# rodrigo-paganini/kalman-vae

Hardware: AMD Instinct MI355X
Metric: sequences/sec (ELBO training step, 32x32xT bouncing-ball) (higher is better)
Workload: dtype f32; 1 GPU; BASELINE configs[1] (configs[2] per-GPU shard): bouncing-ball 32x32, T=50, batch=256/GPU, dynamics=lstm K=3, z=4, u=4, a=2, full train step (fwd incl. sigmoid(x_logits) + loss incl. active-unit stats + bwd + clip + Adam); both the GPU leg and the cpu_baseline leg do this work; preset=c2, global_batch=256, seq_len=50, parallelism=dp1, capture=hipgraph, loss_finite=True, dist_backend=none

## Files before the change

kalman-vae_amd/csrc/kvae_vae.hip:

```cpp
#include <hip/hip_runtime.h>

#include <stdint.h>
#include <stdio.h>
#include <stdlib.h>
#include <string.h>

#include "../../include/kvae_lgssm.h"

namespace kvae {}
using namespace kvae;

extern "C" int kvae_launch_status(const char *what);
static int launch_status(const char *what) { return kvae_launch_status(what); }

#include "vae_epilogue.h"

__device__ __forceinline__ void colsum_v4_body(const float *__restrict__ partials, float *__restrict__ out, int64_t rows, int64_t cols,
                                               unsigned block) {
  __shared__ float4 red[8][64];
  const int lane = threadIdx.x & 63, wv = threadIdx.x >> 6;
  const int64_t c = ((int64_t)block * 64 + lane) * 4;
  float4 s0 = make_float4(0.f, 0.f, 0.f, 0.f), s1 = s0, s2 = s0, s3 = s0;
  if (c < cols) {
    const float *p = partials + c;
// ... 86 lines not shown
    epi_fwd_elem(s, in, bias, out, o, relu);
}

__global__ __launch_bounds__(256) void k_vae_epilogue_bwd_bias(const float *__restrict__ g_out, const float *__restrict__ out,
                                                               float *__restrict__ g_in, float *__restrict__ bias_partials,
                                                               EpiShape s, int n_per_chunk, int relu) {
  extern __shared__ float bins[];
  const int Cin = s.C * s.r * s.r;
  const int OW = s.W * s.r, OH = s.H * s.r;
  const int64_t vol = (int64_t)s.C * OH * OW;
  for (int i = threadIdx.x; i < Cin; i += 256) bins[i] = 0.f;
  __syncthreads();
  const int64_t pos = (int64_t)blockIdx.x * 256 + threadIdx.x;
  if (pos < vol) {
    const int ow = (int)(pos % OW);
    const int oh = (int)((pos / OW) % OH);
    const int c = (int)(pos / ((int64_t)OW * OH));
    const int ch = c * s.r * s.r + (oh % s.r) * s.r + (ow % s.r);
    const int64_t in_off = ((int64_t)ch * s.H + oh / s.r) * s.W + ow / s.r;
    const int64_t in_vol = (int64_t)Cin * s.H * s.W;
    const int64_t n0 = (int64_t)blockIdx.y * n_per_chunk;
    const int64_t n1 = n0 + n_per_chunk < s.N ? n0 + n_per_chunk : s.N;
    float acc = 0.f;
    for (int64_t n = n0; n < n1; ++n) {
      float g = g_out[n * vol + pos];
      if (relu && !(out[n * vol + pos] > 0.f)) g = 0.f;
      g_in[n * in_vol + in_off] = g;
      acc += g;
    }
    atomicAdd(&bins[ch], acc);
  }
  __syncthreads();
  for (int i = threadIdx.x; i < Cin; i += 256) {
    if (bins[i] != 0.f) atomicAdd(&bias_partials[(int64_t)blockIdx.y * Cin + i], bins[i]);
  }
}

__global__ __launch_bounds__(256) void k_vae_epilogue_bwd(const float *g_out, const float *out, float *g_in, EpiShape s,
                                                          int64_t total, int relu) {
  for (int64_t o = (int64_t)blockIdx.x * 256 + threadIdx.x; o < total; o += (int64_t)gridDim.x * 256)
    epi_bwd_elem(s, g_out, out, g_in, o, relu);
}

#define KVAE_EPI_SAMPLES_PER_CHUNK 32
extern "C" int64_t kvae_bias_partial_rows(int64_t N);
static unsigned epi_grid(int64_t total) {
  const int64_t blocks = (total + 255) / 256;
  return (unsigned)(blocks < 256 * 32 ? blocks : 256 * 32);
}

extern "C" {
int kvae_bias_shuffle_act_fwd(const float *in, const float *bias, float *out, int64_t N, int32_t C, int32_t H, int32_t W,
                              int32_t r, int32_t relu, void *stream) {
  if (!in || !bias || !out) return KVAE_ERR_NULL;
  if (N < 1 || C < 1 || H < 1 || W < 1 || r < 1) return KVAE_ERR_ARG;
  const EpiShape s{N, C, H, W, r};
  const int64_t total = N * C * H * W * r * r;
  const bool aligned = ((uintptr_t)in % 16 == 0) && ((uintptr_t)out % 16 == 0);
  if (aligned && r == 1 && W % 4 == 0)
    k_vae_epilogue_fwd_v4<1><<<dim3(epi_grid(total / 4)), dim3(256), 0, (hipStream_t)stream>>>(in, bias, out, C, H, W, total / 4, relu);
  else if (aligned && r == 2 && W % 2 == 0)
    k_vae_epilogue_fwd_v4<2><<<dim3(epi_grid(total / 4)), dim3(256), 0, (hipStream_t)stream>>>(in, bias, out, C, H, W, total / 4, relu);
  else
    k_vae_epilogue_fwd<<<dim3(epi_grid(total)), dim3(256), 0, (hipStream_t)stream>>>(in, bias, out, s, total, relu);
  return launch_status("k_vae_epilogue_fwd");
}
int kvae_bias_shuffle_act_bwd(const float *g_out, const float *out, float *g_in, float *bias_partials, int64_t N, int32_t C,
                              int32_t H, int32_t W, int32_t r, int32_t relu, void *stream) {
  if (!g_out || !g_in || (relu && !out)) return KVAE_ERR_NULL;
  if (N < 1 || C < 1 || H < 1 || W < 1 || r < 1) return KVAE_ERR_ARG;
  const EpiShape s{N, C, H, W, r};
  const int64_t total = N * C * H * W * r * r;
  hipStream_t st = (hipStream_t)stream;
  if (bias_partials) {
    const int Cin = C * r * r;
    const int64_t chunks = kvae_bias_partial_rows(N);
    if (hipMemsetAsync(bias_partials, 0, sizeof(float) * chunks * Cin, st) != hipSuccess) return launch_status("memset bias_partials");
    const int64_t vol = (int64_t)C * H * W * r * r;
    k_vae_epilogue_bwd_bias<<<dim3((unsigned)((vol + 255) / 256), (unsigned)chunks), dim3(256), sizeof(float) * Cin, st>>>(
        g_out, out, g_in, bias_partials, s, KVAE_EPI_SAMPLES_PER_CHUNK, relu);
    return launch_status("k_vae_epilogue_bwd_bias");
  }
  k_vae_epilogue_bwd<<<dim3(epi_grid(total)), dim3(256), 0, st>>>(g_out, out, g_in, s, total, relu);
  return launch_status("k_vae_epilogue_bwd");
}
int kvae_colsum(const float *partials, float *out, int64_t rows, int64_t cols, void *stream) {
  if (!partials || !out) return KVAE_ERR_NULL;
  if (rows < 1 || cols < 1) return KVAE_ERR_ARG;
  if ((cols & 3) == 0 && ((((uintptr_t)partials | (uintptr_t)out) & 15) == 0))
    k_colsum_v4<<<dim3((unsigned)((cols + 255) / 256)), dim3(512), 0, (hipStream_t)stream>>>(partials, out, rows, cols);
  else
    k_colsum<<<dim3((unsigned)((cols + 63) / 64)), dim3(256), 0, (hipStream_t)stream>>>(partials, out, rows, cols);
  return launch_status("k_colsum");
}
int kvae_colsum2(const float *pa, float *oa, int64_t rows_a, int64_t cols_a, const float *pb, float *ob, int64_t rows_b,
                 int64_t cols_b, void *stream) {
  if (!pa || !oa || !pb || !ob) return KVAE_ERR_NULL;
  if (rows_a < 1 || cols_a < 1 || rows_b < 1 || cols_b < 1) return KVAE_ERR_ARG;
  if (((cols_a | cols_b) & 3) == 0 && ((((uintptr_t)pa | (uintptr_t)oa | (uintptr_t)pb | (uintptr_t)ob) & 15) == 0)) {
    const unsigned nb_a = (unsigned)((cols_a + 255) / 256), nb_b = (unsigned)((cols_b + 255) / 256);
    k_colsum_v4_pair<<<dim3(nb_a + nb_b), dim3(512), 0, (hipStream_t)stream>>>(pa, oa, rows_a, cols_a, nb_a, pb, ob, rows_b, cols_b);
    return launch_status("k_colsum_v4_pair");
  }
  const int rc = kvae_colsum(pa, oa, rows_a, cols_a, stream);
  return rc ? rc : kvae_colsum(pb, ob, rows_b, cols_b, stream);
}
int64_t kvae_bias_partial_rows(int64_t N) { return (N + KVAE_EPI_SAMPLES_PER_CHUNK - 1) / KVAE_EPI_SAMPLES_PER_CHUNK; }
}

constexpr int CA_BLOCKS = 512;
constexpr int CA_MAX_SEG = 1024;
__global__ __launch_bounds__(256) void k_grad_sumsq(const float *__restrict__ g, int64_t n, const int32_t *__restrict__ seg_of,
                                                    int n_seg, const float *__restrict__ seg_active,
                                                    const float *__restrict__ div_dev, float *__restrict__ seg_steps,
                                                    float *__restrict__ ws) {
  __shared__ float red[256];
  const float inv = div_dev ? 1.0f / fmaxf(*div_dev, 1.0f) : 1.0f;
  const bool gated = seg_of && seg_active;
  float s = 0.f;
  for (int64_t i = (int64_t)blockIdx.x * 256 + threadIdx.x; i < n; i += (int64_t)gridDim.x * 256) {
    float v = g[i] * inv;
    if (gated && seg_active[seg_of[i]] == 0.f) v = 0.f;
    s = fmaf(v, v, s);
  }
  red[threadIdx.x] = s;
  __syncthreads();
  for (int o = 128; o > 0; o >>= 1) {
    if ((int)threadIdx.x < o) red[threadIdx.x] += red[threadIdx.x + o];
    __syncthreads();
  }
  if (threadIdx.x == 0) ws[blockIdx.x] = red[0];
  if (blockIdx.x == 0)
    for (int sg = threadIdx.x; sg < n_seg; sg += 256)
      if (!seg_active || seg_active[sg] != 0.f) seg_steps[sg] += 1.0f;
}
__global__ __launch_bounds__(256) void k_clip_adam(float *__restrict__ p, const float *__restrict__ g, float *__restrict__ m,
                                                   float *__restrict__ v, int64_t n, const int32_t *__restrict__ seg_of, int n_seg,
                                                   const float *__restrict__ seg_active, const float *__restrict__ seg_steps,
                                                   const float *__restrict__ lr_dev, float lr, float beta1, float beta2, float eps,
                                                   float wd, float clip, const float *__restrict__ div_dev,
                                                   float *__restrict__ norm_out, const float *__restrict__ ws, int nparts) {
  __shared__ float red[256];
  __shared__ float s_step_size[CA_MAX_SEG], s_bc2s[CA_MAX_SEG];
  float s = 0.f;
  for (int i = threadIdx.x; i < nparts; i += 256) s += ws[i];
  red[threadIdx.x] = s;
  const float lrv = lr_dev ? *lr_dev : lr;
  for (int sg = threadIdx.x; sg < n_seg; sg += 256) {
    const float step = seg_steps[sg];
    const bool on = !seg_active || seg_active[sg] != 0.f;
    s_step_size[sg] = on ? lrv / (1.0f - powf(beta1, step)) : -1.0f;
    s_bc2s[sg] = on ? sqrtf(1.0f - powf(beta2, step)) : 1.0f;
  }
  __syncthreads();
  for (int o = 128; o > 0; o >>= 1) {
    if ((int)threadIdx.x < o) red[threadIdx.x] += red[threadIdx.x + o];
    __syncthreads();
  }
  const float total = sqrtf(red[0]);
  if (norm_out && blockIdx.x == 0 && threadIdx.x == 0) *norm_out = total;
  const float inv = div_dev ? 1.0f / fmaxf(*div_dev, 1.0f) : 1.0f;
  const float scale = inv * (clip > 0.f ? fminf(clip / (total + 1e-6f), 1.0f) : 1.0f);
  for (int64_t i = (int64_t)blockIdx.x * 256 + threadIdx.x; i < n; i += (int64_t)gridDim.x * 256) {
    const int sg = seg_of ? seg_of[i] : 0;
    const float step_size = s_step_size[sg], bc2s = s_bc2s[sg];
    if (step_size < 0.f) continue;
    float gi = g[i] * scale;
    const float pi = p[i];
    if (wd != 0.f) gi = fmaf(wd, pi, gi);
    const float mi = m[i] + (gi - m[i]) * (1.0f - beta1);
    const float vi = beta2 * v[i] + (1.0f - beta2) * gi * gi;
    m[i] = mi, v[i] = vi;
    p[i] = pi - step_size * mi / (sqrtf(vi) / bc2s + eps);
  }
}
extern "C" int kvae_clip_adam(float *params, const float *grads, float *exp_avg, float *exp_avg_sq, int64_t n,
                              const int32_t *seg_of, int32_t n_seg, const float *seg_active, float *seg_steps, const float *lr_dev,
                              float lr, float beta1, float beta2, float eps, float weight_decay, float clip, const float *div_dev,
                              float *norm_out, float *ws, void *stream) {
  if (!params || !grads || !exp_avg || !exp_avg_sq || !seg_steps || !ws) return KVAE_ERR_NULL;
  if (n < 1 || n_seg < 1 || n_seg > CA_MAX_SEG || (!seg_of && n_seg != 1)) return KVAE_ERR_ARG;
  const int64_t want = (n + 1023) / 1024;
  const unsigned parts = (unsigned)(want < CA_BLOCKS ? want : CA_BLOCKS);
  k_grad_sumsq<<<dim3(parts), dim3(256), 0, (hipStream_t)stream>>>(grads, n, seg_of, n_seg, seg_active, div_dev, seg_steps, ws);
  int rc = launch_status("k_grad_sumsq");
  if (rc) return rc;
  const unsigned blocks = (unsigned)((n + 255) / 256 < 2048 ? (n + 255) / 256 : 2048);
  k_clip_adam<<<dim3(blocks), dim3(256), 0, (hipStream_t)stream>>>(params, grads, exp_avg, exp_avg_sq, n, seg_of, n_seg, seg_active,
                                                                   seg_steps, lr_dev, lr, beta1, beta2, eps, weight_decay, clip,
                                                                   div_dev, norm_out, ws, (int)parts);
  return launch_status("k_clip_adam");
}

#include "vae_loss.h"

__global__ __launch_bounds__(256) void k_vae_bce_fwd(const float *__restrict__ logits, const float *__restrict__ x,
                                                     float *__restrict__ frame_ll, int64_t frames, int pixels) {
  const int64_t f = (int64_t)blockIdx.x * 4 + (threadIdx.x >> 6);
  const int lane = threadIdx.x & 63;
  if (f >= frames) return;
  const float *l = logits + f * pixels, *t = x + f * pixels;
  float acc = 0.f;
  if ((pixels & 3) == 0 && (((uintptr_t)l | (uintptr_t)t) & 15) == 0) {
    for (int i = lane * 4; i < pixels; i += 256) {
      const float4 a = *reinterpret_cast<const float4 *>(l + i), b = *reinterpret_cast<const float4 *>(t + i);
      acc += bce_logit(a.x, b.x) + bce_logit(a.y, b.y) + bce_logit(a.z, b.z) + bce_logit(a.w, b.w);
    }
  } else {
    for (int i = lane; i < pixels; i += 64) acc += bce_logit(l[i], t[i]);
  }
  for (int off = 32; off > 0; off >>= 1) acc += __shfl_down(acc, off, 64);
  if (lane == 0) frame_ll[f] = -acc;
}

__global__ __launch_bounds__(256) void k_vae_bce_bwd(const float *__restrict__ logits, const float *__restrict__ x,
                                                     const float *__restrict__ g_frame, float *__restrict__ g_logits,
                                                     int64_t total, int pixels) {
  for (int64_t i = ((int64_t)blockIdx.x * 256 + threadIdx.x) * 4; i < total; i += (int64_t)gridDim.x * 1024) {
    const float g = -g_frame[i / pixels];
    const float4 a = *reinterpret_cast<const float4 *>(logits + i), b = *reinterpret_cast<const float4 *>(x + i);
    *reinterpret_cast<float4 *>(g_logits + i) = make_float4(g * (sigmoid_stable(a.x) - b.x), g * (sigmoid_stable(a.y) - b.y),
                                                            g * (sigmoid_stable(a.z) - b.z), g * (sigmoid_stable(a.w) - b.w));
  }
}
__global__ __launch_bounds__(256) void k_vae_bce_bwd_scalar(const float *logits, const float *x, const float *g_frame,
                                                            float *g_logits, int64_t total, int pixels) {
  for (int64_t i = (int64_t)blockIdx.x * 256 + threadIdx.x; i < total; i += (int64_t)gridDim.x * 256)
    g_logits[i] = -g_frame[i / pixels] * (sigmoid_stable(logits[i]) - x[i]);
}

extern "C" {
int kvae_bce_frames_fwd(const float *logits, const float *x, float *frame_ll, int64_t frames, int32_t pixels, void *stream) {
  if (!logits || !x || !frame_ll) return KVAE_ERR_NULL;
  if (frames < 1 || pixels < 1) return KVAE_ERR_ARG;
  k_vae_bce_fwd<<<dim3((unsigned)((frames + 3) / 4)), dim3(256), 0, (hipStream_t)stream>>>(logits, x, frame_ll, frames, pixels);
  return launch_status("k_vae_bce_fwd");
}
int kvae_bce_frames_bwd(const float *logits, const float *x, const float *g_frame, float *g_logits, int64_t frames,
                        int32_t pixels, void *stream) {
  if (!logits || !x || !g_frame || !g_logits) return KVAE_ERR_NULL;
  if (frames < 1 || pixels < 1) return KVAE_ERR_ARG;
  const int64_t total = frames * pixels;
  const bool v4 = (pixels & 3) == 0 && ((((uintptr_t)logits | (uintptr_t)x | (uintptr_t)g_logits) & 15) == 0);
  if (v4)
    k_vae_bce_bwd<<<dim3(epi_grid(total / 4)), dim3(256), 0, (hipStream_t)stream>>>(logits, x, g_frame, g_logits, total, pixels);
  else
    k_vae_bce_bwd_scalar<<<dim3(epi_grid(total)), dim3(256), 0, (hipStream_t)stream>>>(logits, x, g_frame, g_logits, total, pixels);
  return launch_status("k_vae_bce_bwd");
}
}

#include "vae_conv_edge.h"
extern "C" {
int64_t kvae_conv_edge_partial_rows(int64_t N) { return N < 1024 ? (N < 1 ? 1 : N) : 1024; }

int kvae_dec_head_fwd(const float *in, const float *W, const float *bias, float *logits, float *w_scratch, int64_t N,
                      int32_t Cin, int32_t side, void *stream) {
  if (!in || !W || !bias || !logits || !w_scratch) return KVAE_ERR_NULL;
  if (N < 1) return KVAE_ERR_ARG;
  if (Cin != DH_CI || side != DH_S) return KVAE_ERR_DIMS;
  k_dec_head_prep<<<dim3(1), dim3(256), 0, (hipStream_t)stream>>>(W, w_scratch);
  k_dec_head_fwd<<<dim3((unsigned)N), dim3(256), 0, (hipStream_t)stream>>>(in, w_scratch, bias, logits);
  return launch_status("k_dec_head_fwd");
}
int kvae_dec_head_bwd(const float *in, const float *W, const float *g_logits, float *g_in, float *w_partials,
                      float *b_partials, float *w_scratch, int64_t N, int32_t Cin, int32_t side, void *stream) {
  if (!in || !W || !g_logits || !w_partials || !b_partials || !w_scratch) return KVAE_ERR_NULL;
  if (N < 1) return KVAE_ERR_ARG;
  if (Cin != DH_CI || side != DH_S) return KVAE_ERR_DIMS;
  if (g_in) {
    k_dec_head_prep<<<dim3(1), dim3(256), 0, (hipStream_t)stream>>>(W, w_scratch);
    k_dec_head_bwd_data<<<dim3((unsigned)N), dim3(256), 0, (hipStream_t)stream>>>(g_logits, w_scratch, g_in);
    const int rc = launch_status("k_dec_head_bwd_data");
    if (rc) return rc;
  }
  k_dec_head_wrw<<<dim3((unsigned)kvae_conv_edge_partial_rows(N)), dim3(256), 0, (hipStream_t)stream>>>(in, g_logits, w_partials,
                                                                                                     b_partials, N);
  return launch_status("k_dec_head_wrw");
}
int kvae_enc_stem_fwd(const float *x, const float *W, const float *bias, float *out, uint32_t *relu_bits, int64_t N, int32_t Cout,
                      int32_t side, void *stream) {
  if (!x || !W || !bias || !out) return KVAE_ERR_NULL;
  if (N < 1) return KVAE_ERR_ARG;
  if (Cout != ES_CO || side != ES_IN) return KVAE_ERR_DIMS;
  k_enc_stem_fwd<<<dim3((unsigned)N), dim3(256), 0, (hipStream_t)stream>>>(x, W, bias, out, relu_bits);
  return launch_status("k_enc_stem_fwd");
}
int kvae_enc_stem_bwd(const float *x, const float *out, const uint32_t *relu_bits, const float *g_out, float *w_partials,
                      float *b_partials, int64_t N, int32_t Cout, int32_t side, void *stream) {
  if (!x || (!out && !relu_bits) || !g_out || !w_partials || !b_partials) return KVAE_ERR_NULL;
  if (N < 1) return KVAE_ERR_ARG;
  if (Cout != ES_CO || side != ES_IN) return KVAE_ERR_DIMS;
  static const int mfma = getenv("KVAE_STEM_MFMA") ? atoi(getenv("KVAE_STEM_MFMA")) : 1;
  const dim3 grid((unsigned)kvae_conv_edge_partial_rows(N));
  if (mfma == 1 && relu_bits) k_enc_stem_wrw_mfma<true><<<grid, dim3(256), 0, (hipStream_t)stream>>>(x, out, relu_bits, g_out, w_partials, b_partials, N);
  else if (!out) return KVAE_ERR_NULL;
  else if (mfma) k_enc_stem_wrw_mfma<false><<<grid, dim3(256), 0, (hipStream_t)stream>>>(x, out, relu_bits, g_out, w_partials, b_partials, N);
  else k_enc_stem_wrw<<<grid, dim3(256), 0, (hipStream_t)stream>>>(x, out, g_out, w_partials, b_partials, N);
  return launch_status("k_enc_stem_wrw");
}
}

#include "vae_conv_mid.h"
static inline int64_t enc_mid_grid(int64_t N, int32_t side) {
  const int64_t fpi = side == 16 ? 2 : 8, iters = (N + fpi - 1) / fpi;
  return iters < 256 ? (iters < 1 ? 1 : iters) : 256;
}
extern "C" {
int64_t kvae_enc_mid_partial_rows(int64_t N, int32_t side) { return enc_mid_grid(N, side); }

int kvae_enc_mid_fwd(const float *in, const float *W, const float *bias, float *out, int64_t N, int32_t C, int32_t side,
                     void *stream) {
  if (!in || !W || !bias || !out) return KVAE_ERR_NULL;
  if (N < 1 || (N + 256 * 8) * EM_C * side * side * 4 >= EM_MAX_BYTES) return KVAE_ERR_ARG;
  if (C != EM_C || (side != 16 && side != 8)) return KVAE_ERR_DIMS;
  const dim3 grid((unsigned)enc_mid_grid(N, side));
  if (side == 16) k_enc_mid_fwd<16><<<grid, dim3(256), 0, (hipStream_t)stream>>>(in, W, bias, out, N);
  else k_enc_mid_fwd<8><<<grid, dim3(256), 0, (hipStream_t)stream>>>(in, W, bias, out, N);
  return launch_status("k_enc_mid_fwd");
}
int kvae_enc_mid_bwd(const float *in, const float *W, const float *out, const float *g_out, float *g_in,
                     float *w_partials, float *b_partials, int64_t N, int32_t C, int32_t side, void *stream) {
  if (!in || !W || !out || !g_out || !w_partials || !b_partials) return KVAE_ERR_NULL;
  if (N < 1 || (N + 256 * 8) * EM_C * side * side * 4 >= EM_MAX_BYTES) return KVAE_ERR_ARG;
  if (C != EM_C || (side != 16 && side != 8)) return KVAE_ERR_DIMS;
  const dim3 grid((unsigned)enc_mid_grid(N, side));
  if (g_in) {
    if (side == 16) k_enc_mid_bwd_data<16><<<grid, dim3(256), 0, (hipStream_t)stream>>>(W, out, g_out, g_in, N);
    else k_enc_mid_bwd_data<8><<<grid, dim3(256), 0, (hipStream_t)stream>>>(W, out, g_out, g_in, N);
    const int rc = launch_status("k_enc_mid_bwd_data");
    if (rc) return rc;
  }
  if (side == 16) k_enc_mid_wrw<16><<<grid, dim3(256), 0, (hipStream_t)stream>>>(in, out, g_out, w_partials, b_partials, N);
  else k_enc_mid_wrw<8><<<grid, dim3(256), 0, (hipStream_t)stream>>>(in, out, g_out, w_partials, b_partials, N);
  return launch_status("k_enc_mid_wrw");
}
}

#include "vae_conv_up_wino.h"
static bool dec_up_wino() {
  static const int env = getenv("KVAE_WINO") ? atoi(getenv("KVAE_WINO")) : 1;
  return env != 0;
}
static int g_dec_up_wgs = 0;
static inline int64_t dec_up_cap() {
  static const int env = getenv("KVAE_UP_WGS") ? atoi(getenv("KVAE_UP_WGS")) : 0;
  const int v = env >= 1 && env <= 256 ? env : __atomic_load_n(&g_dec_up_wgs, __ATOMIC_RELAXED);
  return v >= 1 && v <= 256 ? v : 256;
}
static inline int64_t dec_up_grid(int64_t N, int32_t side) {
  const int64_t fpi = side == 8 ? 2 : 8, iters = (N + fpi - 1) / fpi, cap = dec_up_cap();
  return iters < cap ? (iters < 1 ? 1 : iters) : cap;
}
extern "C" {
int64_t kvae_dec_up_partial_rows(int64_t N, int32_t side) { return dec_up_grid(N, side); }
int32_t kvae_dec_up_set_workgroups(int32_t n) {
  const int32_t prev = (int32_t)dec_up_cap();
  __atomic_store_n(&g_dec_up_wgs, n >= 1 && n <= 256 ? n : 0, __ATOMIC_RELAXED);
  return prev;
}

int kvae_dec_up_fwd(const float *x, const float *W, const float *bias, float *out, int64_t N, int32_t Cin, int32_t side,
                    void *stream) {
  if (!x || !W || !bias || !out) return KVAE_ERR_NULL;
  if (N < 1 || (N + 256 * 8) * UP_CO * side * side * 4 >= EM_MAX_BYTES) return KVAE_ERR_ARG;
  if (Cin != UP_CI || (side != 8 && side != 4)) return KVAE_ERR_DIMS;
  const dim3 grid((unsigned)dec_up_grid(N, side));
  if (dec_up_wino()) {
    const int64_t sets = side == 8 ? N : (N + 3) / 4;
    const dim3 wgrid((unsigned)(sets < dec_up_cap() ? sets : dec_up_cap()));
    if (side == 8) k_dec_up_fwd_wino<8><<<wgrid, dim3(512), 0, (hipStream_t)stream>>>(x, W, bias, out, N);
    else k_dec_up_fwd_wino<4><<<wgrid, dim3(512), 0, (hipStream_t)stream>>>(x, W, bias, out, N);
    return launch_status("k_dec_up_fwd_wino");
  }
  if (side == 8) k_dec_up_fwd<8><<<grid, dim3(256), 0, (hipStream_t)stream>>>(x, W, bias, out, N);
  else k_dec_up_fwd<4><<<grid, dim3(256), 0, (hipStream_t)stream>>>(x, W, bias, out, N);
  return launch_status("k_dec_up_fwd");
}
int kvae_dec_up_bwd(const float *x, const float *W, const float *out, const float *g_out, float *g_x, float *w_partials,
                    float *b_partials, int64_t N, int32_t Cin, int32_t side, void *stream) {
  if (!x || !W || !out || !g_out || !w_partials || !b_partials) return KVAE_ERR_NULL;
  if (N < 1 || (N + 256 * 8) * UP_CO * side * side * 4 >= EM_MAX_BYTES) return KVAE_ERR_ARG;
  if (Cin != UP_CI || (side != 8 && side != 4)) return KVAE_ERR_DIMS;
  const dim3 grid((unsigned)dec_up_grid(N, side));
  if (g_x) {
    const int64_t sets = side == 8 ? N : (N + 3) / 4;
    const dim3 wgrid((unsigned)(sets < dec_up_cap() ? sets : dec_up_cap()));
    if (dec_up_wino() && side == 8) k_dec_up_bwd_data_wino<8><<<wgrid, dim3(512), 0, (hipStream_t)stream>>>(W, out, g_out, g_x, N);
    else if (dec_up_wino()) k_dec_up_bwd_data_wino<4><<<wgrid, dim3(512), 0, (hipStream_t)stream>>>(W, out, g_out, g_x, N);
    else if (side == 8) k_dec_up_bwd_data<8><<<grid, dim3(256), 0, (hipStream_t)stream>>>(W, out, g_out, g_x, N);
    else k_dec_up_bwd_data<4><<<grid, dim3(256), 0, (hipStream_t)stream>>>(W, out, g_out, g_x, N);
    const int rc = launch_status("k_dec_up_bwd_data");
    if (rc) return rc;
  }
  if (dec_up_wino()) {
    if (side == 8) k_dec_up_wrw_wino<8><<<grid, dim3(512), 0, (hipStream_t)stream>>>(x, out, g_out, w_partials, b_partials, N);
    else k_dec_up_wrw_wino<4><<<grid, dim3(512), 0, (hipStream_t)stream>>>(x, out, g_out, w_partials, b_partials, N);
    return launch_status("k_dec_up_wrw_wino");
  }
  if (side == 8) k_dec_up_wrw<8><<<grid, dim3(256), 0, (hipStream_t)stream>>>(x, out, g_out, w_partials, b_partials, N);
  else k_dec_up_wrw<4><<<grid, dim3(256), 0, (hipStream_t)stream>>>(x, out, g_out, w_partials, b_partials, N);
  return launch_status("k_dec_up_wrw");
}
}

#include "vae_heads.h"
extern "C" {
int64_t kvae_head_partial_rows(void) { return HD_WAVES; }

int kvae_enc_head_fwd(const float *feat, const float *Wmu, const float *bmu, const float *Wvar, const float *bvar,
                      const float *eps, float *mu, float *var, float *a, int64_t N, int32_t F, int32_t A,
                      float noise_emission, void *stream) {
  if (!feat || !Wmu || !bmu || !Wvar || !bvar || !mu || !var || !a) return KVAE_ERR_NULL;
  if (N < 1) return KVAE_ERR_ARG;
  if (F != HD_F || A != HD_A) return KVAE_ERR_DIMS;
  const unsigned grid = (unsigned)(N < 4 * 512 ? (N + 3) / 4 : 512);
  k_enc_head_fwd<<<dim3(grid), dim3(256), 0, (hipStream_t)stream>>>(feat, Wmu, bmu, Wvar, bvar, eps, noise_emission, mu, var, a, N);
  return launch_status("k_enc_head_fwd");
}
int kvae_enc_head_bwd(const float *feat, const float *Wmu, const float *Wvar, const float *var, const float *eps,
                      const float *g_a, const float *g_mu, const float *g_var, float *g_feat, float *w_partials,
                      float *b_partials, int64_t N, int32_t F, int32_t A, float noise_emission, void *stream) {
  if (!feat || !Wmu || !Wvar || !var || !g_feat || !w_partials || !b_partials) return KVAE_ERR_NULL;
  if (N < 1) return KVAE_ERR_ARG;
  if (F != HD_F || A != HD_A) return KVAE_ERR_DIMS;
  k_enc_head_bwd<<<dim3(HD_WAVES / 4), dim3(256), 0, (hipStream_t)stream>>>(feat, Wmu, Wvar, var, eps, g_a, g_mu, g_var,
                                                                             noise_emission, g_feat, w_partials, b_partials, N);
  return launch_status("k_enc_head_bwd");
}
int kvae_dec_fc_fwd(const float *a, const float *W, const float *b, float *h, int64_t N, int32_t F, int32_t A, void *stream) {
  if (!a || !W || !b || !h) return KVAE_ERR_NULL;
  if (N < 1) return KVAE_ERR_ARG;
  if (F != HD_F || A != HD_A) return KVAE_ERR_DIMS;
  k_dec_fc_fwd<<<dim3(epi_grid(N * (HD_F / 4))), dim3(256), 0, (hipStream_t)stream>>>(a, W, b, h, N * (HD_F / 4));
  return launch_status("k_dec_fc_fwd");
}
int kvae_dec_fc_bwd(const float *g_h, const float *a, const float *W, float *g_a, float *w_partials, float *b_partials,
                    int64_t N, int32_t F, int32_t A, void *stream) {
  if (!g_h || !a || !W || !g_a || !w_partials || !b_partials) return KVAE_ERR_NULL;
  if (N < 1) return KVAE_ERR_ARG;
  if (F != HD_F || A != HD_A) return KVAE_ERR_DIMS;
  k_dec_fc_bwd<<<dim3(HD_WAVES / 4), dim3(256), 0, (hipStream_t)stream>>>(g_h, a, W, g_a, w_partials, b_partials, N);
  return launch_status("k_dec_fc_bwd");
}
int kvae_latent_reg_fwd(const float *a, const float *mu, const float *var, float *reg, int64_t N, int32_t A, void *stream) {
  if (!a || !mu || !var || !reg) return KVAE_ERR_NULL;
  if (N < 1 || A < 1) return KVAE_ERR_ARG;
  k_latent_reg_fwd<<<dim3(epi_grid(N)), dim3(256), 0, (hipStream_t)stream>>>(a, mu, var, reg, N, A);
  return launch_status("k_latent_reg_fwd");
}
int kvae_latent_reg_bwd(const float *a, const float *mu, const float *var, const float *g, float *g_a, float *g_mu,
                        float *g_var, int64_t N, int32_t A, void *stream) {
  if (!a || !mu || !var || !g || !g_a || !g_mu || !g_var) return KVAE_ERR_NULL;
  if (N < 1 || A < 1) return KVAE_ERR_ARG;
  k_latent_reg_bwd<<<dim3(epi_grid(N * A)), dim3(256), 0, (hipStream_t)stream>>>(a, mu, var, g, g_a, g_mu, g_var, N, A);
  return launch_status("k_latent_reg_bwd");
}
int kvae_loss_head_fwd(const float *lpx, const float *regf, const float *mask, const float *elbo_kf, const float *beta,
                       float scale_reconstruction, float vae_weight, float kf_weight, const float *weights_dev, float *out6,
                       float *coef3, int64_t n, void *stream) {
  if (!lpx || !regf || !elbo_kf || !beta || !out6 || !coef3) return KVAE_ERR_NULL;
  if (n < 1) return KVAE_ERR_ARG;
  k_loss_head_fwd<<<dim3(1), dim3(1024), 0, (hipStream_t)stream>>>(lpx, regf, mask, elbo_kf, beta, scale_reconstruction, vae_weight,
                                                                  kf_weight, weights_dev, out6, coef3, n);
  return launch_status("k_loss_head_fwd");
}
int kvae_loss_head_bwd(const float *g_loss, const float *coef3, const float *mask, float *g_lpx, float *g_regf,
                       float *g_elbo_kf, int64_t n, void *stream) {
  if (!g_loss || !coef3 || !g_lpx || !g_regf || !g_elbo_kf) return KVAE_ERR_NULL;
  if (n < 1) return KVAE_ERR_ARG;
  k_loss_head_bwd<<<dim3(epi_grid(n)), dim3(256), 0, (hipStream_t)stream>>>(g_loss, coef3, mask, g_lpx, g_regf,
                                                                            g_elbo_kf, n);
  return launch_status("k_loss_head_bwd");
}
}
```

kalman-vae_amd/csrc/vae_conv_mid.h:

```cpp
#pragma once
#include <hip/hip_runtime.h>
#include <stdint.h>

namespace kvae {

typedef float em_f16 __attribute__((ext_vector_type(16)));
constexpr int EM_C = 32, EM_W = EM_C * EM_C * 9;

template <int S>
struct EmDims {
  static constexpr int OS = S / 2, PF = OS * OS;
  static constexpr int FPI = 128 / PF;
  static constexpr int PLANE = S * S, FRAME = EM_C * PLANE;
  static constexpr int IT_IN = FPI * FRAME;
  static constexpr int IT_OUT = FPI * EM_C * PF;
};

__device__ __forceinline__ void em_load_weights(float *Wl, const float *__restrict__ W, bool m_is_co) {
  for (int i = threadIdx.x; i < EM_W; i += 256) {
    const int tap = i >> 10, k = (i >> 5) & 31, m = i & 31;
    const int co = m_is_co ? m : k, ci = m_is_co ? k : m;
    Wl[i] = W[(co * EM_C + ci) * 9 + tap];
  }
}

constexpr int EM_OOB = 1 << 24;
constexpr int64_t EM_MAX_BYTES = (int64_t)1 << 31;

typedef unsigned int em_u4 __attribute__((ext_vector_type(4)));
__device__ __forceinline__ __amdgpu_buffer_rsrc_t em_rsrc(const void *p, int64_t bytes) {
  return __builtin_amdgcn_make_buffer_rsrc(const_cast<void *>(p), 0, (int)bytes, 0x00020000);
}
__device__ __forceinline__ float4 em_ld4(__amdgpu_buffer_rsrc_t r, uint32_t byte_off) {
  const em_u4 v = __builtin_amdgcn_raw_buffer_load_b128(r, byte_off, 0, 0);
  return make_float4(__uint_as_float(v.x), __uint_as_float(v.y), __uint_as_float(v.z), __uint_as_float(v.w));
}
__device__ __forceinline__ void em_st4(__amdgpu_buffer_rsrc_t r, uint32_t byte_off, const float4 v) {
  const em_u4 u = {__float_as_uint(v.x), __float_as_uint(v.y), __float_as_uint(v.z), __float_as_uint(v.w)};
  __builtin_amdgcn_raw_buffer_store_b128(u, r, byte_off, 0, 0);
}
__device__ __forceinline__ void em_st1(__amdgpu_buffer_rsrc_t r, uint32_t byte_off, float v) {
  __builtin_amdgcn_raw_buffer_store_b32(__float_as_uint(v), r, byte_off, 0, 0);
}
#ifdef KVAE_EM_STAMPS
__device__ unsigned long long em_stamps[4096];
#define EM_STAMP(slot, k) do { if (blockIdx.x == 0 && threadIdx.x == 0 && (slot) < 500) em_stamps[(slot) * 8 + (k)] = __builtin_amdgcn_s_memtime(); } while (0)
#else
#define EM_STAMP(slot, k) do {} while (0)
#endif
#define KV_MFMA_F32(a, b, c) __builtin_amdgcn_mfma_f32_32x32x2f32((a), (b), (c), 0, 0, 0)
#define KV_ACC_ROW(r, half) (((r) & 3) + 8 * ((r) >> 2) + 4 * (half))

template <int S>
__global__ __launch_bounds__(256) void k_enc_mid_fwd(const float *__restrict__ in, const float *__restrict__ W,
                                                     const float *__restrict__ bias, float *__restrict__ out, int64_t N) {
  using D = EmDims<S>;
  __shared__ float lds[EM_W + D::IT_IN + D::IT_OUT];
  float *Wl = lds, *fr = lds + EM_W, *ot = fr + D::IT_IN;
  const int tid = threadIdx.x, lane = tid & 63, wv = tid >> 6, q = lane & 31, half = lane >> 5;
  em_load_weights(Wl, W, true);
  const int64_t iters = (N + D::FPI - 1) / D::FPI, total = N * D::FRAME;
  const int gp = 32 * wv + q, fl = gp / D::PF, pix = gp % D::PF, oh = pix / D::OS, ow = pix % D::OS;
  const bool top = oh == 0, left = ow == 0;
  const int bbase = fl * D::FRAME + half * D::PLANE + (2 * oh - 1) * S + (2 * ow - 1);
  const int b_t = top ? EM_OOB : bbase, b_l = left ? EM_OOB : bbase, b_tl = (top || left) ? EM_OOB : bbase;
  const int abase = half * 32 + q;
  float bv[16];
#pragma unroll
  for (int r = 0; r < 16; ++r) bv[r] = bias[KV_ACC_ROW(r, half)];

  const int rot = blockIdx.x & 15;
  const __amdgpu_buffer_rsrc_t rin = em_rsrc(in, total * 4), rout = em_rsrc(out, N * EM_C * D::PF * 4);
  float4 pre[16];
  int64_t it = blockIdx.x;
  auto fetch1 = [&](int64_t i, int j) {
    pre[j] = em_ld4(rin, (uint32_t)(i * D::IT_IN + (tid + 256 * ((j + rot) & 15)) * 4) * 4u);
  };
  uint32_t done_base = 0x80000000u;
  auto flush1 = [&](int j) {
    em_st4(rout, done_base + (uint32_t)(tid + 256 * j) * 16u, reinterpret_cast<const float4 *>(ot)[tid + 256 * j]);
  };
#pragma unroll
  for (int j = 0; j < 16; ++j) fetch1(it, j);
  for (int slot = 0; it < iters; it += gridDim.x, ++slot) {
    EM_STAMP(slot, 0);
    __syncthreads();
    EM_STAMP(slot, 1);
#pragma unroll
    for (int j = 0; j < 16; ++j) reinterpret_cast<float4 *>(fr)[tid + 256 * ((j + rot) & 15)] = pre[j];
    EM_STAMP(slot, 2);
    __syncthreads();
    EM_STAMP(slot, 3);
    EM_STAMP(slot, 4);
    em_f16 acc;
#pragma unroll
    for (int r = 0; r < 16; ++r) acc[r] = 0.f;
    float av[36][4], bw[36][4];
    auto rd = [&](int g) {
#pragma unroll
      for (int u = 0; u < 4; ++u) {
        const int k = g * 4 + u, tap = k / 16, jj = k % 16, ky = tap / 3, kx = tap % 3;
        av[g][u] = Wl[abase + (tap * 32 + 2 * jj) * 32];
        bw[g][u] = fr[(ky == 0 ? (kx == 0 ? b_tl : b_t) : (kx == 0 ? b_l : bbase)) + ky * S + kx + 2 * jj * D::PLANE];
      }
    };
    rd(0);
    rd(1);
#pragma unroll
    for (int g = 0; g < 36; ++g) {
      if (g + 2 < 36) rd(g + 2);
      if (g < 4) flush1(g);
      else if (g < 20) fetch1(it + gridDim.x, g - 4);
      __builtin_amdgcn_sched_barrier(0);
#pragma unroll
      for (int u = 0; u < 4; ++u) acc = KV_MFMA_F32(av[g][u], bw[g][u], acc);
      __builtin_amdgcn_sched_barrier(0);
    }
    EM_STAMP(slot, 5);
    __syncthreads();
    EM_STAMP(slot, 6);
#pragma unroll
    for (int r = 0; r < 16; ++r) ot[(fl * EM_C + KV_ACC_ROW(r, half)) * D::PF + pix] = fmaxf(acc[r] + bv[r], 0.f);
    EM_STAMP(slot, 7);
    done_base = (uint32_t)(it * D::IT_OUT) * 4u;
  }
  __syncthreads();
#pragma unroll
  for (int j = 0; j < 4; ++j) flush1(j);
}

template <int S>
__global__ __launch_bounds__(256) void k_enc_mid_bwd_data(const float *__restrict__ W, const float *__restrict__ out,
                                                          const float *__restrict__ g_out, float *__restrict__ g_in, int64_t N) {
  using D = EmDims<S>;
  __shared__ float lds[EM_W + D::IT_OUT + D::IT_IN];
  float *Wl = lds, *gm = lds + EM_W, *ot = gm + D::IT_OUT;
  const int tid = threadIdx.x, lane = tid & 63, wv = tid >> 6, q = lane & 31, half = lane >> 5;
  em_load_weights(Wl, W, false);
  const int64_t iters = (N + D::FPI - 1) / D::FPI, total_in = N * D::FRAME, total_out = N * EM_C * D::PF;
  const int cp = 32 * wv + q, fl = cp / D::PF, idx = cp % D::PF, a_ = idx / D::OS, b_ = idx % D::OS;
  const bool bottom = a_ == D::OS - 1, right = b_ == D::OS - 1;
  const int gbase = fl * EM_C * D::PF + half * D::PF + a_ * D::OS + b_;
  const int g_b = bottom ? EM_OOB : gbase, g_r = right ? EM_OOB : gbase, g_br = (bottom || right) ? EM_OOB : gbase;
  const int abase = half * 32 + q;
  const int obase = fl * D::FRAME + (2 * a_) * S + 2 * b_;

  const int rot = blockIdx.x & 15;
  const __amdgpu_buffer_rsrc_t rg = em_rsrc(g_out, total_out * 4), ro = em_rsrc(out, total_out * 4),
                               rgi = em_rsrc(g_in, total_in * 4);
  float4 pg[4], po[4];
  int64_t it = blockIdx.x;
  auto fetch1 = [&](int64_t i, int j) {
    const uint32_t e = (uint32_t)(i * D::IT_OUT + (tid + 256 * (((j & 3) + rot) & 3)) * 4) * 4u;
    if (j < 4) pg[j] = em_ld4(rg, e);
    else po[j - 4] = em_ld4(ro, e);
  };
  uint32_t done_base = 0x80000000u;
  auto flush1 = [&](int j) {
    const int c = (j + rot) & 15;
    em_st4(rgi, done_base + (uint32_t)(tid + 256 * c) * 16u, reinterpret_cast<const float4 *>(ot)[tid + 256 * c]);
  };
#pragma unroll
  for (int j = 0; j < 8; ++j) fetch1(it, j);
  for (; it < iters; it += gridDim.x) {
    __syncthreads();
#pragma unroll
    for (int j = 0; j < 4; ++j)
      reinterpret_cast<float4 *>(gm)[tid + 256 * ((j + rot) & 3)] =
          make_float4(po[j].x > 0.f ? pg[j].x : 0.f, po[j].y > 0.f ? pg[j].y : 0.f, po[j].z > 0.f ? pg[j].z : 0.f,
                      po[j].w > 0.f ? pg[j].w : 0.f);
    __syncthreads();
    constexpr int E_CLS[9] = {3, 3, 3, 3, 1, 1, 2, 2, 0};
    constexpr int E_KY[9] = {0, 0, 2, 2, 1, 1, 0, 2, 1};
    constexpr int E_KX[9] = {0, 2, 0, 2, 0, 2, 1, 1, 1};
    float av[36][4], bw[36][4];
    auto rd = [&](int g) {
#pragma unroll
      for (int u = 0; u < 4; ++u) {
        const int en = g / 4, jj = (g % 4) * 4 + u, ph = E_CLS[en] >> 1, pw = E_CLS[en] & 1;
        const int dy = (ph == 1 && E_KY[en] == 0) ? 1 : 0, dx = (pw == 1 && E_KX[en] == 0) ? 1 : 0;
        av[g][u] = Wl[abase + ((E_KY[en] * 3 + E_KX[en]) * 32 + 2 * jj) * 32];
        bw[g][u] = gm[(dy ? (dx ? g_br : g_b) : (dx ? g_r : gbase)) + 2 * jj * D::PF + dy * D::OS + dx];
      }
    };
    rd(0);
    rd(1);
    em_f16 acc;
#pragma unroll
    for (int g = 0; g < 36; ++g) {
      const int en = g / 4, cls = E_CLS[en], ph = cls >> 1, pw = cls & 1;
      if (g % 4 == 0 && (en == 0 || E_CLS[en - 1] != cls)) {
#pragma unroll
        for (int r = 0; r < 16; ++r) acc[r] = 0.f;
      }
      if (g + 2 < 36) rd(g + 2);
      if (g < 16) flush1(g);
      else if (g < 24) fetch1(it + gridDim.x, g - 16);
      __builtin_amdgcn_sched_barrier(0);
#pragma unroll
      for (int u = 0; u < 4; ++u) acc = KV_MFMA_F32(av[g][u], bw[g][u], acc);
      __builtin_amdgcn_sched_barrier(0);
      if (g % 4 == 3 && (en == 8 || E_CLS[en + 1] != cls)) {
        if (g == 15) __syncthreads();
#pragma unroll
        for (int r = 0; r < 16; ++r) ot[obase + KV_ACC_ROW(r, half) * D::PLANE + ph * S + pw] = acc[r];
      }
    }
    done_base = (uint32_t)(it * D::IT_IN) * 4u;
  }
  __syncthreads();
#pragma unroll
  for (int j = 0; j < 16; ++j) flush1(j);
}

template <int S>
__global__ __launch_bounds__(256) void k_enc_mid_wrw(const float *__restrict__ in, const float *__restrict__ out,
                                                     const float *__restrict__ g_out, float *__restrict__ w_partials,
                                                     float *__restrict__ b_partials, int64_t N) {
  using D = EmDims<S>;
  constexpr int CSP = D::PLANE + 1, GSP = D::PF + 1;
  __shared__ float lds[D::FPI * EM_C * GSP + D::FPI * EM_C * CSP];
  float *gm = lds, *xin = lds + D::FPI * EM_C * GSP;
  const int tid = threadIdx.x, lane = tid & 63, wv = tid >> 6, q = lane & 31, half = lane >> 5;
  const int64_t iters = (N + D::FPI - 1) / D::FPI, total_in = N * D::FRAME, total_out = N * EM_C * D::PF;
  const int wframe = S == 16 ? (wv >> 1) : 2 * wv, wpix0 = S == 16 ? 32 * (wv & 1) : 0;
  const int oh0 = wpix0 / D::OS;
  const int abase = wframe * EM_C * GSP + q * GSP + wpix0 + half;
  const int bbase = wframe * EM_C * CSP + q * CSP + (2 * oh0 - 1) * S - 1 + 2 * half;
  const bool wtop = oh0 == 0, wleft = half == 0;
  const int x_t = wtop ? EM_OOB : bbase, x_l = wleft ? EM_OOB : bbase, x_tl = (wtop || wleft) ? EM_OOB : bbase;

  em_f16 acc[9];
#pragma unroll
  for (int t = 0; t < 9; ++t)
#pragma unroll
    for (int r = 0; r < 16; ++r) acc[t][r] = 0.f;
  float bsum = 0.f;

  const int rot = blockIdx.x & 15;
  const __amdgpu_buffer_rsrc_t rin = em_rsrc(in, total_in * 4), rg = em_rsrc(g_out, total_out * 4),
                               ro = em_rsrc(out, total_out * 4);
  float4 px[16], pg[4], po[4];
  int64_t it = blockIdx.x;
  const int tin = S == 16 ? ((lane >> 4) << 6) | (wv << 4) | (lane & 15) : tid;
  auto fetch1 = [&](int64_t i, int j) {
    if (j < 16) {
      px[j] = em_ld4(rin, (uint32_t)(i * D::IT_IN + (tin + 256 * ((j + rot) & 15)) * 4) * 4u);
    } else {
      const uint32_t e = (uint32_t)(i * D::IT_OUT + (tid + 256 * (((j & 3) + rot) & 3)) * 4) * 4u;
      if (j < 20) pg[j - 16] = em_ld4(rg, e);
      else po[j - 20] = em_ld4(ro, e);
    }
  };
#pragma unroll
  for (int j = 0; j < 24; ++j) fetch1(it, j);
  for (; it < iters; it += gridDim.x) {
    __syncthreads();
#pragma unroll
    for (int j = 0; j < 16; ++j) {
      const int e = (tin + 256 * ((j + rot) & 15)) * 4, f = e / D::FRAME, c = (e % D::FRAME) / D::PLANE, p = e % D::PLANE;
      float *d = xin + (f * EM_C + c) * CSP + p;
      d[0] = px[j].x; d[1] = px[j].y; d[2] = px[j].z; d[3] = px[j].w;
    }
#pragma unroll
    for (int j = 0; j < 4; ++j) {
      const int e = (tid + 256 * ((j + rot) & 3)) * 4, f = e / (EM_C * D::PF), c = (e / D::PF) % EM_C, p = e % D::PF;
      float *d = gm + (f * EM_C + c) * GSP + p;
      d[0] = po[j].x > 0.f ? pg[j].x : 0.f; d[1] = po[j].y > 0.f ? pg[j].y : 0.f;
      d[2] = po[j].z > 0.f ? pg[j].z : 0.f; d[3] = po[j].w > 0.f ? pg[j].w : 0.f;
    }
    __syncthreads();
    float av[16], bw[16][9];
    auto rd = [&](int i) {
      const int fi = S == 16 ? 0 : i / 8, p = S == 16 ? 2 * i : 2 * (i % 8);
      const int ohr = p / D::OS, owr = p % D::OS;
      av[i] = gm[abase + fi * EM_C * GSP + p];
#pragma unroll
      for (int tap = 0; tap < 9; ++tap) {
        const bool zt = tap / 3 == 0 && ohr == 0, zl = tap % 3 == 0 && owr == 0;
        bw[i][tap] = xin[(zt ? (zl ? x_tl : x_t) : (zl ? x_l : bbase)) + fi * EM_C * CSP + (2 * ohr + tap / 3) * S + 2 * owr + tap % 3];
      }
    };
    rd(0);
#pragma unroll
    for (int i = 0; i < 16; ++i) {
      if (i + 1 < 16) rd(i + 1);
      if (i < 12) {
        fetch1(it + gridDim.x, 2 * i);
        fetch1(it + gridDim.x, 2 * i + 1);
      }
      __builtin_amdgcn_sched_barrier(0);
      bsum += av[i];
#pragma unroll
      for (int tap = 0; tap < 9; ++tap) acc[tap] = KV_MFMA_F32(av[i], bw[i][tap], acc[tap]);
      __builtin_amdgcn_sched_barrier(0);
    }
  }
  float *red = lds, *redb = lds + EM_W;
  for (int w = 0; w < 4; ++w) {
    __syncthreads();
    if (wv == w) {
#pragma unroll
      for (int tap = 0; tap < 9; ++tap)
#pragma unroll
        for (int r = 0; r < 16; ++r) {
          float *d = red + (KV_ACC_ROW(r, half) * EM_C + q) * 9 + tap;
          *d = w == 0 ? acc[tap][r] : *d + acc[tap][r];
        }
      float *db = redb + half * EM_C + q;
      *db = w == 0 ? bsum : *db + bsum;
    }
  }
  __syncthreads();
  for (int i = tid; i < EM_W; i += 256) w_partials[(int64_t)blockIdx.x * EM_W + i] = red[i];
  if (tid < EM_C) b_partials[(int64_t)blockIdx.x * EM_C + tid] = redb[tid] + redb[EM_C + tid];
}

}
```

Before: 94950 sequences/s.

## Halve enc-mid backward LDS footprint and double workgroups for two-per-CU occupancy

The backward-data kernel now keeps its weights in registers, loaded once through the output staging buffer, so the weight region no longer occupies LDS. The weight-gradient kernel processes half as many frames per iteration, which halves its LDS planes and prefetch registers. Both kernels declare launch bounds for two workgroups per CU, and the grid cap for the backward kernels doubles to 512. Prefetch bases past the end are clamped to an out-of-range offset. The intent is better latency hiding through occupancy, paid for with 144 weight registers per thread in bwd_data and more partial rows for the weight-gradient reduction.

New measurement: 95450 sequences/s (median of 6 runs). About the same (+0.5%).

```diff
diff --git a/kalman-vae_amd/csrc/kvae_vae.hip b/kalman-vae_amd/csrc/kvae_vae.hip
--- a/kalman-vae_amd/csrc/kvae_vae.hip
+++ b/kalman-vae_amd/csrc/kvae_vae.hip
@@ -412,19 +412,24 @@
 }
 
 #include "vae_conv_mid.h"
-static inline int64_t enc_mid_grid(int64_t N, int32_t side) {
-  const int64_t fpi = side == 16 ? 2 : 8, iters = (N + fpi - 1) / fpi;
-  return iters < 256 ? (iters < 1 ? 1 : iters) : 256;
+enum EmKernel { EM_FWD, EM_BWD_DATA, EM_WRW };
+static inline int64_t enc_mid_cap(EmKernel k) {
+  static const int env = getenv("KVAE_EM_WGS") ? atoi(getenv("KVAE_EM_WGS")) : 2;
+  return 256 * (k == EM_FWD || env == 1 ? 1 : 2);
+}
+static inline int64_t enc_mid_grid(int64_t N, int32_t side, EmKernel k) {
+  const int64_t fpi = (side == 16 ? 2 : 8) / (k == EM_WRW ? 2 : 1), iters = (N + fpi - 1) / fpi, cap = enc_mid_cap(k);
+  return iters < cap ? (iters < 1 ? 1 : iters) : cap;
 }
 extern "C" {
-int64_t kvae_enc_mid_partial_rows(int64_t N, int32_t side) { return enc_mid_grid(N, side); }
+int64_t kvae_enc_mid_partial_rows(int64_t N, int32_t side) { return enc_mid_grid(N, side, EM_WRW); }
 
 int kvae_enc_mid_fwd(const float *in, const float *W, const float *bias, float *out, int64_t N, int32_t C, int32_t side,
                      void *stream) {
   if (!in || !W || !bias || !out) return KVAE_ERR_NULL;
   if (N < 1 || (N + 256 * 8) * EM_C * side * side * 4 >= EM_MAX_BYTES) return KVAE_ERR_ARG;
   if (C != EM_C || (side != 16 && side != 8)) return KVAE_ERR_DIMS;
-  const dim3 grid((unsigned)enc_mid_grid(N, side));
+  const dim3 grid((unsigned)enc_mid_grid(N, side, EM_FWD));
   if (side == 16) k_enc_mid_fwd<16><<<grid, dim3(256), 0, (hipStream_t)stream>>>(in, W, bias, out, N);
   else k_enc_mid_fwd<8><<<grid, dim3(256), 0, (hipStream_t)stream>>>(in, W, bias, out, N);
   return launch_status("k_enc_mid_fwd");
@@ -434,15 +439,15 @@
   if (!in || !W || !out || !g_out || !w_partials || !b_partials) return KVAE_ERR_NULL;
   if (N < 1 || (N + 256 * 8) * EM_C * side * side * 4 >= EM_MAX_BYTES) return KVAE_ERR_ARG;
   if (C != EM_C || (side != 16 && side != 8)) return KVAE_ERR_DIMS;
-  const dim3 grid((unsigned)enc_mid_grid(N, side));
+  const dim3 grid((unsigned)enc_mid_grid(N, side, EM_BWD_DATA)), wgrid((unsigned)enc_mid_grid(N, side, EM_WRW));
   if (g_in) {
     if (side == 16) k_enc_mid_bwd_data<16><<<grid, dim3(256), 0, (hipStream_t)stream>>>(W, out, g_out, g_in, N);
     else k_enc_mid_bwd_data<8><<<grid, dim3(256), 0, (hipStream_t)stream>>>(W, out, g_out, g_in, N);
     const int rc = launch_status("k_enc_mid_bwd_data");
     if (rc) return rc;
   }
-  if (side == 16) k_enc_mid_wrw<16><<<grid, dim3(256), 0, (hipStream_t)stream>>>(in, out, g_out, w_partials, b_partials, N);
-  else k_enc_mid_wrw<8><<<grid, dim3(256), 0, (hipStream_t)stream>>>(in, out, g_out, w_partials, b_partials, N);
+  if (side == 16) k_enc_mid_wrw<16><<<wgrid, dim3(256), 0, (hipStream_t)stream>>>(in, out, g_out, w_partials, b_partials, N);
+  else k_enc_mid_wrw<8><<<wgrid, dim3(256), 0, (hipStream_t)stream>>>(in, out, g_out, w_partials, b_partials, N);
   return launch_status("k_enc_mid_wrw");
 }
 }
diff --git a/kalman-vae_amd/csrc/vae_conv_mid.h b/kalman-vae_amd/csrc/vae_conv_mid.h
--- a/kalman-vae_amd/csrc/vae_conv_mid.h
+++ b/kalman-vae_amd/csrc/vae_conv_mid.h
@@ -14,6 +14,8 @@
   static constexpr int PLANE = S * S, FRAME = EM_C * PLANE;
   static constexpr int IT_IN = FPI * FRAME;
   static constexpr int IT_OUT = FPI * EM_C * PF;
+  static constexpr int FPW = FPI / 2;
+  static constexpr int PS_IN = IT_IN / 2, PS_OUT = IT_OUT / 2;
 };
 
 __device__ __forceinline__ void em_load_weights(float *Wl, const float *__restrict__ W, bool m_is_co) {
@@ -24,7 +26,16 @@
   }
 }
 
+__device__ __forceinline__ void em_weights_to_regs(float (&wr)[144], const float *Wl, int abase) {
+#pragma unroll
+  for (int k = 0; k < 144; ++k) wr[k] = Wl[abase + ((k / 16) * 32 + 2 * (k % 16)) * 32];
+}
+
 constexpr int EM_OOB = 1 << 24;
+constexpr uint32_t EM_PAST = 0x80000000u;
+__device__ __forceinline__ uint32_t em_next_base(int64_t i, int64_t iters, int floats) {
+  return i < iters ? (uint32_t)(i * floats) * 4u : EM_PAST;
+}
 constexpr int64_t EM_MAX_BYTES = (int64_t)1 << 31;
 
 typedef unsigned int em_u4 __attribute__((ext_vector_type(4)));
@@ -130,19 +141,17 @@
 }
 
 template <int S>
-__global__ __launch_bounds__(256) void k_enc_mid_bwd_data(const float *__restrict__ W, const float *__restrict__ out,
+__global__ __launch_bounds__(256, 2) void k_enc_mid_bwd_data(const float *__restrict__ W, const float *__restrict__ out,
                                                           const float *__restrict__ g_out, float *__restrict__ g_in, int64_t N) {
   using D = EmDims<S>;
-  __shared__ float lds[EM_W + D::IT_OUT + D::IT_IN];
-  float *Wl = lds, *gm = lds + EM_W, *ot = gm + D::IT_OUT;
+  __shared__ float lds[D::IT_OUT + D::IT_IN];
+  float *gm = lds, *ot = gm + D::IT_OUT;
   const int tid = threadIdx.x, lane = tid & 63, wv = tid >> 6, q = lane & 31, half = lane >> 5;
-  em_load_weights(Wl, W, false);
   const int64_t iters = (N + D::FPI - 1) / D::FPI, total_in = N * D::FRAME, total_out = N * EM_C * D::PF;
   const int cp = 32 * wv + q, fl = cp / D::PF, idx = cp % D::PF, a_ = idx / D::OS, b_ = idx % D::OS;
   const bool bottom = a_ == D::OS - 1, right = b_ == D::OS - 1;
   const int gbase = fl * EM_C * D::PF + half * D::PF + a_ * D::OS + b_;
   const int g_b = bottom ? EM_OOB : gbase, g_r = right ? EM_OOB : gbase, g_br = (bottom || right) ? EM_OOB : gbase;
-  const int abase = half * 32 + q;
   const int obase = fl * D::FRAME + (2 * a_) * S + 2 * b_;
 
   const int rot = blockIdx.x & 15;
@@ -150,19 +159,24 @@
                                rgi = em_rsrc(g_in, total_in * 4);
   float4 pg[4], po[4];
   int64_t it = blockIdx.x;
-  auto fetch1 = [&](int64_t i, int j) {
-    const uint32_t e = (uint32_t)(i * D::IT_OUT + (tid + 256 * (((j & 3) + rot) & 3)) * 4) * 4u;
+  auto fetch1 = [&](uint32_t base, int j) {
+    const uint32_t e = base + (uint32_t)(tid + 256 * (((j & 3) + rot) & 3)) * 16u;
     if (j < 4) pg[j] = em_ld4(rg, e);
     else po[j - 4] = em_ld4(ro, e);
   };
-  uint32_t done_base = 0x80000000u;
+  uint32_t done_base = EM_PAST;
   auto flush1 = [&](int j) {
     const int c = (j + rot) & 15;
     em_st4(rgi, done_base + (uint32_t)(tid + 256 * c) * 16u, reinterpret_cast<const float4 *>(ot)[tid + 256 * c]);
   };
 #pragma unroll
-  for (int j = 0; j < 8; ++j) fetch1(it, j);
+  for (int j = 0; j < 8; ++j) fetch1(em_next_base(it, iters, D::IT_OUT), j);
+  float wr[144];
+  em_load_weights(ot, W, false);
+  __syncthreads();
+  em_weights_to_regs(wr, ot, half * 32 + q);
   for (; it < iters; it += gridDim.x) {
+    const uint32_t next_base = em_next_base(it + gridDim.x, iters, D::IT_OUT);
     __syncthreads();
 #pragma unroll
     for (int j = 0; j < 4; ++j)
@@ -173,13 +187,12 @@
     constexpr int E_CLS[9] = {3, 3, 3, 3, 1, 1, 2, 2, 0};
     constexpr int E_KY[9] = {0, 0, 2, 2, 1, 1, 0, 2, 1};
     constexpr int E_KX[9] = {0, 2, 0, 2, 0, 2, 1, 1, 1};
-    float av[36][4], bw[36][4];
+    float bw[36][4];
     auto rd = [&](int g) {
 #pragma unroll
       for (int u = 0; u < 4; ++u) {
         const int en = g / 4, jj = (g % 4) * 4 + u, ph = E_CLS[en] >> 1, pw = E_CLS[en] & 1;
         const int dy = (ph == 1 && E_KY[en] == 0) ? 1 : 0, dx = (pw == 1 && E_KX[en] == 0) ? 1 : 0;
-        av[g][u] = Wl[abase + ((E_KY[en] * 3 + E_KX[en]) * 32 + 2 * jj) * 32];
         bw[g][u] = gm[(dy ? (dx ? g_br : g_b) : (dx ? g_r : gbase)) + 2 * jj * D::PF + dy * D::OS + dx];
       }
     };
@@ -195,10 +208,11 @@
       }
       if (g + 2 < 36) rd(g + 2);
       if (g < 16) flush1(g);
-      else if (g < 24) fetch1(it + gridDim.x, g - 16);
-      __builtin_amdgcn_sched_barrier(0);
-#pragma unroll
-      for (int u = 0; u < 4; ++u) acc = KV_MFMA_F32(av[g][u], bw[g][u], acc);
+      else if (g < 24) fetch1(next_base, g - 16);
+      __builtin_amdgcn_sched_barrier(0);
+#pragma unroll
+      for (int u = 0; u < 4; ++u)
+        acc = KV_MFMA_F32(wr[(E_KY[en] * 3 + E_KX[en]) * 16 + (g % 4) * 4 + u], bw[g][u], acc);
       __builtin_amdgcn_sched_barrier(0);
       if (g % 4 == 3 && (en == 8 || E_CLS[en + 1] != cls)) {
         if (g == 15) __syncthreads();
@@ -214,16 +228,17 @@
 }
 
 template <int S>
-__global__ __launch_bounds__(256) void k_enc_mid_wrw(const float *__restrict__ in, const float *__restrict__ out,
+__global__ __launch_bounds__(256, 2) void k_enc_mid_wrw(const float *__restrict__ in, const float *__restrict__ out,
                                                      const float *__restrict__ g_out, float *__restrict__ w_partials,
                                                      float *__restrict__ b_partials, int64_t N) {
   using D = EmDims<S>;
   constexpr int CSP = D::PLANE + 1, GSP = D::PF + 1;
-  __shared__ float lds[D::FPI * EM_C * GSP + D::FPI * EM_C * CSP];
-  float *gm = lds, *xin = lds + D::FPI * EM_C * GSP;
+  static_assert(D::FPW * EM_C * (GSP + CSP) >= EM_W + 2 * EM_C, "the fold at the end reuses the planes");
+  __shared__ float lds[D::FPW * EM_C * GSP + D::FPW * EM_C * CSP];
+  float *gm = lds, *xin = lds + D::FPW * EM_C * GSP;
   const int tid = threadIdx.x, lane = tid & 63, wv = tid >> 6, q = lane & 31, half = lane >> 5;
-  const int64_t iters = (N + D::FPI - 1) / D::FPI, total_in = N * D::FRAME, total_out = N * EM_C * D::PF;
-  const int wframe = S == 16 ? (wv >> 1) : 2 * wv, wpix0 = S == 16 ? 32 * (wv & 1) : 0;
+  const int64_t iters = (N + D::FPW - 1) / D::FPW, total_in = N * D::FRAME, total_out = N * EM_C * D::PF;
+  const int wframe = S == 16 ? 0 : wv, wpix0 = S == 16 ? 16 * wv : 0;
   const int oh0 = wpix0 / D::OS;
   const int abase = wframe * EM_C * GSP + q * GSP + wpix0 + half;
   const int bbase = wframe * EM_C * CSP + q * CSP + (2 * oh0 - 1) * S - 1 + 2 * half;
@@ -240,54 +255,55 @@
   const int rot = blockIdx.x & 15;
   const __amdgpu_buffer_rsrc_t rin = em_rsrc(in, total_in * 4), rg = em_rsrc(g_out, total_out * 4),
                                ro = em_rsrc(out, total_out * 4);
-  float4 px[16], pg[4], po[4];
+  float4 px[8], pg[2], po[2];
   int64_t it = blockIdx.x;
   const int tin = S == 16 ? ((lane >> 4) << 6) | (wv << 4) | (lane & 15) : tid;
-  auto fetch1 = [&](int64_t i, int j) {
-    if (j < 16) {
-      px[j] = em_ld4(rin, (uint32_t)(i * D::IT_IN + (tin + 256 * ((j + rot) & 15)) * 4) * 4u);
+  auto fetch1 = [&](uint32_t base_in, uint32_t base_out, int j) {
+    if (j < 8) {
+      px[j] = em_ld4(rin, base_in + (uint32_t)(tin + 256 * ((j + rot) & 7)) * 16u);
     } else {
-      const uint32_t e = (uint32_t)(i * D::IT_OUT + (tid + 256 * (((j & 3) + rot) & 3)) * 4) * 4u;
-      if (j < 20) pg[j - 16] = em_ld4(rg, e);
-      else po[j - 20] = em_ld4(ro, e);
-    }
-  };
-#pragma unroll
-  for (int j = 0; j < 24; ++j) fetch1(it, j);
+      const uint32_t e = base_out + (uint32_t)(tid + 256 * (((j & 1) + rot) & 1)) * 16u;
+      if (j < 10) pg[j - 8] = em_ld4(rg, e);
+      else po[j - 10] = em_ld4(ro, e);
+    }
+  };
+#pragma unroll
+  for (int j = 0; j < 12; ++j) fetch1(em_next_base(it, iters, D::PS_IN), em_next_base(it, iters, D::PS_OUT), j);
   for (; it < iters; it += gridDim.x) {
-    __syncthreads();
-#pragma unroll
-    for (int j = 0; j < 16; ++j) {
-      const int e = (tin + 256 * ((j + rot) & 15)) * 4, f = e / D::FRAME, c = (e % D::FRAME) / D::PLANE, p = e % D::PLANE;
+    const uint32_t next_in = em_next_base(it + gridDim.x, iters, D::PS_IN),
+                   next_out = em_next_base(it + gridDim.x, iters, D::PS_OUT);
+    __syncthreads();
+#pragma unroll
+    for (int j = 0; j < 8; ++j) {
+      const int e = (tin + 256 * ((j + rot) & 7)) * 4, f = e / D::FRAME, c = (e % D::FRAME) / D::PLANE, p = e % D::PLANE;
       float *d = xin + (f * EM_C + c) * CSP + p;
       d[0] = px[j].x; d[1] = px[j].y; d[2] = px[j].z; d[3] = px[j].w;
     }
 #pragma unroll
-    for (int j = 0; j < 4; ++j) {
-      const int e = (tid + 256 * ((j + rot) & 3)) * 4, f = e / (EM_C * D::PF), c = (e / D::PF) % EM_C, p = e % D::PF;
+    for (int j = 0; j < 2; ++j) {
+      const int e = (tid + 256 * ((j + rot) & 1)) * 4, f = e / (EM_C * D::PF), c = (e / D::PF) % EM_C, p = e % D::PF;
       float *d = gm + (f * EM_C + c) * GSP + p;
       d[0] = po[j].x > 0.f ? pg[j].x : 0.f; d[1] = po[j].y > 0.f ? pg[j].y : 0.f;
       d[2] = po[j].z > 0.f ? pg[j].z : 0.f; d[3] = po[j].w > 0.f ? pg[j].w : 0.f;
     }
     __syncthreads();
-    float av[16], bw[16][9];
+    float av[8], bw[8][9];
     auto rd = [&](int i) {
-      const int fi = S == 16 ? 0 : i / 8, p = S == 16 ? 2 * i : 2 * (i % 8);
-      const int ohr = p / D::OS, owr = p % D::OS;
-      av[i] = gm[abase + fi * EM_C * GSP + p];
+      const int p = 2 * i, ohr = p / D::OS, owr = p % D::OS;
+      av[i] = gm[abase + p];
 #pragma unroll
       for (int tap = 0; tap < 9; ++tap) {
         const bool zt = tap / 3 == 0 && ohr == 0, zl = tap % 3 == 0 && owr == 0;
-        bw[i][tap] = xin[(zt ? (zl ? x_tl : x_t) : (zl ? x_l : bbase)) + fi * EM_C * CSP + (2 * ohr + tap / 3) * S + 2 * owr + tap % 3];
+        bw[i][tap] = xin[(zt ? (zl ? x_tl : x_t) : (zl ? x_l : bbase)) + (2 * ohr + tap / 3) * S + 2 * owr + tap % 3];
       }
     };
     rd(0);
 #pragma unroll
-    for (int i = 0; i < 16; ++i) {
-      if (i + 1 < 16) rd(i + 1);
-      if (i < 12) {
-        fetch1(it + gridDim.x, 2 * i);
-        fetch1(it + gridDim.x, 2 * i + 1);
+    for (int i = 0; i < 8; ++i) {
+      if (i + 1 < 8) rd(i + 1);
+      if (i < 6) {
+        fetch1(next_in, next_out, 2 * i);
+        fetch1(next_in, next_out, 2 * i + 1);
       }
       __builtin_amdgcn_sched_barrier(0);
       bsum += av[i];
```
